# cloneofsimo/paint-with-words-sd

Measured on NVIDIA H100. Metric: unet_steps_per_sec_512sq_cfg, higher is better.
Workload: dtype f16

## Files before the change

include/pww_b200.h:

```cpp
#ifndef PWW_B200_H_
#define PWW_B200_H_

#include <stddef.h>
#include <stdint.h>

#ifdef __cplusplus
extern "C" {
#endif

typedef enum {
  PWW_OK = 0,
  PWW_ERR_BAD_ARG = -1,
  PWW_ERR_UNSUPPORTED = -2,
  PWW_ERR_CUDA = -3,
  PWW_ERR_WORKSPACE = -4
} pww_status_t;

#define PWW_STAT_MAX 0
#define PWW_STAT_STD 1

int pww_version(void);

const char* pww_status_str(int status);

// ... 15 lines not shown
                      int B, int H, int N, int T, int D,
                      int64_t q_batch_stride, int64_t q_row_stride,
                      int64_t k_batch_stride, int64_t k_row_stride,
                      int64_t o_batch_stride, int64_t o_row_stride,
                      const float* wmap, int64_t wmap_batch_stride, const int32_t* wmap_index,
                      const float* stats, const float* g_sigma, float scale, void* stream);

size_t pww_xattn_fused_workspace_bytes(void);
int pww_xattn_fused_f16(const void* q, const void* k, const void* v, void* out,
                        int B, int H, int N, int T, int D,
                        int64_t q_batch_stride, int64_t q_row_stride,
                        int64_t k_batch_stride, int64_t k_row_stride,
                        int64_t o_batch_stride, int64_t o_row_stride,
                        const void* mpack, int64_t mpack_batch_stride, int Bw, const int8_t* cidx,
                        const int32_t* wmap_index, int stat, const float* g_sigma, float scale,
                        float* stats, void* workspace, size_t workspace_bytes, void* stream);

int pww_attn_fwd_f16(const void* q, const void* k, const void* v, void* out,
                     int B, int H, int N, int D,
                     int64_t qkv_batch_stride, int64_t qkv_row_stride,
                     int64_t o_batch_stride, int64_t o_row_stride,
                     float scale, void* stream);

size_t pww_groupnorm_workspace_bytes(int B, int HW, int G);
int pww_groupnorm_nhwc_f16(const void* x, const void* add, int64_t add_batch_stride ,
                           const void* gamma, const void* beta, void* y,
                           int B, int HW, int C, int G, float eps, int silu,
                           void* workspace, size_t workspace_bytes, void* stream);

int pww_geglu_f16(const void* in, void* out, int64_t M, int I, void* stream);

int pww_add_layernorm_f16(const void* x, const void* res, const void* gamma, const void* beta, void* sum_out, void* y,
                          int64_t M, int C, float eps, void* stream);

#ifdef __cplusplus
}
#endif
#endif
```

paint_with_words_sd_b200/__init__.py:

```python
from .attention import PwWAttnProcessor, inj_forward, patch_unet, unpatch_all
from .conditioning import (
    _blur_image_mask, _encode_text_color_inputs, _extract_seed_and_sigma_from_context, _get_binary_mask,
    _image_context_seperator, _img_importance_flatten, _tokens_img_attention_weight, always_round,
)
from .pipeline import (
    PaintWithWord_StableDiffusionInpaintPipeline, PaintWithWord_StableDiffusionPipeline, PwWSampler, paint_with_words,
    paint_with_words_inpaint, preprocess, prepare_mask_and_masked_image, pww_load_tools,
)
from .scheduler import LMSDiscreteScheduler
from .weight_function import UnsupportedWeightFunction, WeightFunction, probe_weight_function

__version__ = "0.1.0"
```

paint_with_words_sd_b200/_native.py:

```python
from __future__ import annotations

import ctypes
import os
from typing import Optional

_HERE = os.path.dirname(os.path.abspath(__file__))
LIB_PATH = os.environ.get("PWW_B200_LIB", os.path.join(_HERE, "libpww_b200.so"))

PWW_STAT_MAX, PWW_STAT_STD = 0, 1

EXPORTS = (
    "pww_version", "pww_status_str", "pww_last_cuda_error", "pww_device_supported",
    "pww_xattn_workspace_bytes", "pww_xattn_stats_f16", "pww_xattn_fwd_f16", "pww_attn_fwd_f16",
    "pww_xattn_fused_workspace_bytes", "pww_xattn_fused_f16",
    "pww_groupnorm_workspace_bytes", "pww_groupnorm_nhwc_f16", "pww_geglu_f16", "pww_add_layernorm_f16",
)


class NativeError(RuntimeError):
    pass


_lib: Optional[ctypes.CDLL] = None
launch_count = 0


def lib() -> ctypes.CDLL:
    global _lib
    if _lib is not None:
        return _lib
    if not os.path.exists(LIB_PATH):
        raise NativeError(
            f"{LIB_PATH} not found: build it with `python -m paint_with_words_sd_b200.csrc.build` "
            "(there is no CPU / PyTorch fallback for the attention path)")
    L = ctypes.CDLL(LIB_PATH)
    c_i, c_i64, c_vp, c_f, c_sz = ctypes.c_int, ctypes.c_int64, ctypes.c_void_p, ctypes.c_float, ctypes.c_size_t
    L.pww_version.restype = c_i
    L.pww_status_str.restype = ctypes.c_char_p
    L.pww_status_str.argtypes = [c_i]
    L.pww_last_cuda_error.restype = ctypes.c_char_p
    L.pww_device_supported.restype = c_i
    L.pww_xattn_workspace_bytes.restype = c_sz
    L.pww_xattn_workspace_bytes.argtypes = [c_i] * 5
    L.pww_xattn_stats_f16.restype = c_i
    L.pww_xattn_stats_f16.argtypes = [c_vp, c_vp, c_i, c_i, c_i, c_i, c_i, c_i64, c_i64, c_i64, c_i64, c_i, c_vp,
                                      c_vp, c_vp, c_sz, c_vp]
    L.pww_xattn_fwd_f16.restype = c_i
    L.pww_xattn_fwd_f16.argtypes = [c_vp, c_vp, c_vp, c_vp, c_i, c_i, c_i, c_i, c_i, c_i64, c_i64, c_i64, c_i64,
                                    c_i64, c_i64, c_vp, c_i64, c_vp, c_vp, c_vp, c_f, c_vp]
    L.pww_xattn_fused_workspace_bytes.restype = c_sz
    L.pww_xattn_fused_workspace_bytes.argtypes = []
    L.pww_xattn_fused_f16.restype = c_i
    L.pww_xattn_fused_f16.argtypes = [c_vp, c_vp, c_vp, c_vp, c_i, c_i, c_i, c_i, c_i, c_i64, c_i64, c_i64, c_i64,
                                      c_i64, c_i64, c_vp, c_i64, c_i, c_vp, c_vp, c_i, c_vp, c_f, c_vp, c_vp, c_sz, c_vp]
    L.pww_attn_fwd_f16.restype = c_i
    L.pww_attn_fwd_f16.argtypes = [c_vp, c_vp, c_vp, c_vp, c_i, c_i, c_i, c_i, c_i64, c_i64, c_i64, c_i64, c_f, c_vp]
    L.pww_groupnorm_workspace_bytes.restype = c_sz
    L.pww_groupnorm_workspace_bytes.argtypes = [c_i, c_i, c_i]
    L.pww_groupnorm_nhwc_f16.restype = c_i
    L.pww_groupnorm_nhwc_f16.argtypes = [c_vp, c_vp, c_i64, c_vp, c_vp, c_vp, c_i, c_i, c_i, c_i, c_f, c_i, c_vp, c_sz, c_vp]
    L.pww_geglu_f16.restype = c_i
    L.pww_geglu_f16.argtypes = [c_vp, c_vp, c_i64, c_i, c_vp]
    L.pww_add_layernorm_f16.restype = c_i
    L.pww_add_layernorm_f16.argtypes = [c_vp, c_vp, c_vp, c_vp, c_vp, c_vp, c_i64, c_i, c_f, c_vp]
    _lib = L
    return L


def check(status: int, what: str) -> None:
    if status != 0:
        L = lib()
        msg = L.pww_status_str(status).decode()
        if status == -3:
            msg += ": " + L.pww_last_cuda_error().decode()
        raise NativeError(f"{what} failed: {msg} (status {status})")
```

paint_with_words_sd_b200/csrc/pww_abi.cu:

```cuda
#include <stdio.h>
#include <string.h>

#include "pww_common.cuh"
#include "xattn_tc.cuh"
#include "xattn_fused.cuh"
#include "xattn_fused2.cuh"
#include "attn_tc.cuh"
#include "unet_ops.cuh"
#include <stdlib.h>

namespace {

thread_local char g_last_cuda_error[640] = "";

int cuda_fail(cudaError_t e);

bool aligned16(const void* p) { return (reinterpret_cast<uintptr_t>(p) & 15u) == 0; }

bool supported_head_dim(int D) { return D == 40 || D == 64 || D == 80 || D == 160; }

int check_common(const void* q, const void* k, int B, int H, int N, int T, int D, int64_t q_bs, int64_t q_rs,
                 int64_t k_bs, int64_t k_rs) {
  if (!q || !k || B <= 0 || H <= 0 || N <= 0 || T <= 0 || D <= 0) return PWW_ERR_BAD_ARG;
  if (!aligned16(q) || !aligned16(k)) return PWW_ERR_BAD_ARG;
  if ((q_bs | q_rs | k_bs | k_rs) & 7) return PWW_ERR_BAD_ARG;
  if (q_rs < (int64_t)H * D || k_rs < (int64_t)H * D) return PWW_ERR_BAD_ARG;
  if (!supported_head_dim(D) || T > pww::tc::kTP) return PWW_ERR_UNSUPPORTED;
  return PWW_OK;
}

size_t align_up(size_t x, size_t a) { return (x + a - 1) / a * a; }

int stats_slots_per_image(int, int) { return 2048; }

int cuda_fail(cudaError_t e) {
  snprintf(g_last_cuda_error, sizeof(g_last_cuda_error), "%s: %s %s", cudaGetErrorName(e), cudaGetErrorString(e),
           pww::tc::tc_error_buf());
  pww::tc::tc_error_buf()[0] = 0;
  return PWW_ERR_CUDA;
}

}

extern "C" {

int pww_version(void) { return 100; }

const char* pww_status_str(int status) {
  switch (status) {
    case PWW_OK: return "ok";
    case PWW_ERR_BAD_ARG: return "bad argument (null/misaligned pointer, non-positive size or stride not a multiple of 8)";
    case PWW_ERR_UNSUPPORTED: return "unsupported shape (head dim must be 40/64/80/160, T <= 80)";
    case PWW_ERR_CUDA: return "CUDA error (see pww_last_cuda_error)";
    case PWW_ERR_WORKSPACE: return "workspace too small (see pww_xattn_workspace_bytes)";
    default: return "unknown status";
  }
}

const char* pww_last_cuda_error(void) { return g_last_cuda_error; }

int pww_device_supported(void) {
  int dev = 0, major = 0;
  cudaError_t e = cudaGetDevice(&dev);
  if (e != cudaSuccess) return cuda_fail(e);
  e = cudaDeviceGetAttribute(&major, cudaDevAttrComputeCapabilityMajor, dev);
  if (e != cudaSuccess) return cuda_fail(e);
  return major == 9 ? 1 : 0;
}

// ... 134 lines not shown
    const void* mp = mpack;
    const int8_t* ci = cidx;
    if (mpack && wmap_index) {
      c.wmap_index = wmap_index + b0;
    } else if (mpack) {
      c.wmap_index = nullptr;
      mp = (const __half*)mpack + (int64_t)b0 * mpack_batch_stride;
      ci = cidx + (int64_t)b0 * pww::fx::kTP;
    }
    c.wmap = mpack ? (const float*)mp : nullptr;
    cudaError_t e = cudaErrorInvalidValue;
    switch (D) {
      case 40: e = pww::fx2::launch_fused2<40>(c, mp, mpack_batch_stride, ci, s); break;
      case 64: e = pww::fx2::launch_fused2<64>(c, mp, mpack_batch_stride, ci, s); break;
      case 80: e = pww::fx2::launch_fused2<80>(c, mp, mpack_batch_stride, ci, s); break;
      case 160: e = pww::fx2::launch_fused2<160>(c, mp, mpack_batch_stride, ci, s); break;
    }
    if (e == cudaErrorInvalidConfiguration) return PWW_ERR_UNSUPPORTED;
    if (e != cudaSuccess) return cuda_fail(e);
  }
  return PWW_OK;
}

size_t pww_groupnorm_workspace_bytes(int B, int HW, int G) {
  if (B <= 0 || HW <= 0 || G <= 0) return 0;
  return align_up((size_t)B * sizeof(unsigned int), 256) + align_up((size_t)B * G * 2 * sizeof(float), 256) +
         (size_t)B * pww::uops::gn_chunks(HW) * G * 2 * sizeof(float);
}

int pww_groupnorm_nhwc_f16(const void* x, const void* add, int64_t add_batch_stride, const void* gamma, const void* beta,
                           void* y, int B, int HW, int C, int G, float eps, int silu, void* workspace,
                           size_t workspace_bytes, void* stream) {
  if (!x || !gamma || !beta || !y || !workspace || B <= 0 || HW <= 0 || C <= 0 || G <= 0) return PWW_ERR_BAD_ARG;
  if (!aligned16(x) || !aligned16(y) || !aligned16(gamma) || !aligned16(beta) || (add && !aligned16(add)))
    return PWW_ERR_BAD_ARG;
  if ((C & 7) || (C % G) || G > 64 || (C >> 3) > 1024) return PWW_ERR_UNSUPPORTED;
  if (add && ((add_batch_stride & 7) || add_batch_stride < C)) return PWW_ERR_BAD_ARG;
  if (workspace_bytes < pww_groupnorm_workspace_bytes(B, HW, G)) return PWW_ERR_WORKSPACE;
  pww::uops::GnParams p;
  p.x = (const __half*)x; p.add = (const __half*)add; p.add_bs = add_batch_stride; p.gamma = (const __half*)gamma; p.beta = (const __half*)beta;
  p.y = (__half*)y;
  char* w = (char*)workspace;
  p.counters = (unsigned int*)w;
  w += align_up((size_t)B * sizeof(unsigned int), 256);
  p.stats = (float*)w;
  w += align_up((size_t)B * G * 2 * sizeof(float), 256);
  p.partial = (float*)w;
  p.B = B; p.HW = HW; p.C = C; p.G = G; p.eps = eps; p.silu = silu;
  p.chunks = pww::uops::gn_chunks(HW);
  p.rows_per_chunk = (HW + p.chunks - 1) / p.chunks;
  cudaStream_t s = (cudaStream_t)stream;
  const int nvec = C >> 3;
  const int rpp = nvec >= 256 ? 1 : 256 / nvec;
  const size_t smem1 = (size_t)rpp * C * 2 * sizeof(float);
  if (smem1 > 48 * 1024) return PWW_ERR_UNSUPPORTED;
  pww::uops::gn_stats_kernel<<<dim3(p.chunks, B), nvec * rpp, smem1, s>>>(p);
  int rows_per_block = (int)(((long long)HW * B + 2 * pww::tc::num_sms() - 1) / (2 * pww::tc::num_sms()));
  if (rows_per_block < rpp) rows_per_block = rpp;
  if (rows_per_block > 32) rows_per_block = 32;
  pww::uops::gn_apply_kernel<<<dim3((HW + rows_per_block - 1) / rows_per_block, B), nvec * rpp, 0, s>>>(p, rows_per_block);
  cudaError_t e = cudaGetLastError();
  return e == cudaSuccess ? PWW_OK : cuda_fail(e);
}

int pww_geglu_f16(const void* in, void* out, int64_t M, int I, void* stream) {
  if (!in || !out || M <= 0 || I <= 0 || !aligned16(in) || !aligned16(out)) return PWW_ERR_BAD_ARG;
  if (I & 7) return PWW_ERR_UNSUPPORTED;
  const long long total = (long long)M * (I >> 3);
  long long blocks = (total + 255) / 256;
  const long long cap = (long long)pww::tc::num_sms() * 16;
  if (blocks > cap) blocks = cap;
  pww::uops::geglu_kernel<<<(int)blocks, 256, 0, (cudaStream_t)stream>>>((const __half*)in, (__half*)out, M, I);
  cudaError_t e = cudaGetLastError();
  return e == cudaSuccess ? PWW_OK : cuda_fail(e);
}

int pww_add_layernorm_f16(const void* x, const void* res, const void* gamma, const void* beta, void* sum_out, void* y,
                          int64_t M, int C, float eps, void* stream) {
  if (!x || !gamma || !beta || !y || M <= 0 || C <= 0) return PWW_ERR_BAD_ARG;
  if (!aligned16(x) || !aligned16(y) || !aligned16(gamma) || !aligned16(beta) || (res && !aligned16(res)) ||
      (sum_out && !aligned16(sum_out)))
    return PWW_ERR_BAD_ARG;
  if ((C & 7) || C > 2048) return PWW_ERR_UNSUPPORTED;
// ... 65 lines not shown
```

paint_with_words_sd_b200/csrc/unet_ops.cuh:

```cuda
#pragma once
#include "pww_common.cuh"

namespace pww {
namespace uops {

struct GnParams {
  const __half* x;
  const __half* add;
  long long add_bs;
  const __half* gamma;
  const __half* beta;
  __half* y;
  float* partial;
  float* stats;
  unsigned int* counters;
  int B, HW, C, G, chunks, rows_per_chunk, silu;
  float eps;
};

__global__ void gn_stats_kernel(GnParams p) {
  extern __shared__ float sm[];
  const int nvec = p.C >> 3;
  const int rpp = blockDim.x / nvec;
  const int v = threadIdx.x % nvec, rl = threadIdx.x / nvec;
  const int b = blockIdx.y, chunk = blockIdx.x;
  const int r0 = chunk * p.rows_per_chunk, r1 = min(p.HW, r0 + p.rows_per_chunk);
  float s[8], q[8], a[8];
#pragma unroll
  for (int i = 0; i < 8; ++i) { s[i] = 0.f; q[i] = 0.f; a[i] = 0.f; }
  if (p.add) {
    const uint4 av = *reinterpret_cast<const uint4*>(p.add + (size_t)b * p.add_bs + v * 8);
    const __half2* ah = reinterpret_cast<const __half2*>(&av);
#pragma unroll
    for (int i = 0; i < 4; ++i) { float2 f = __half22float2(ah[i]); a[2 * i] = f.x; a[2 * i + 1] = f.y; }
  }
  const __half* xb = p.x + (size_t)b * p.HW * p.C;
  for (int r = r0 + rl; r < r1; r += 4 * rpp) {
    uint4 xv[4];
#pragma unroll
    for (int u = 0; u < 4; ++u) {
      const int rr = r + u * rpp;
      xv[u] = rr < r1 ? __ldg(reinterpret_cast<const uint4*>(xb + (size_t)rr * p.C) + v) : make_uint4(0, 0, 0, 0);
    }
#pragma unroll
    for (int u = 0; u < 4; ++u) {
      if (r + u * rpp < r1) {
        const __half2* xh = reinterpret_cast<const __half2*>(&xv[u]);
#pragma unroll
        for (int i = 0; i < 4; ++i) {
          float2 f = __half22float2(xh[i]);
          const float x0 = f.x + a[2 * i], x1 = f.y + a[2 * i + 1];
          s[2 * i] += x0; q[2 * i] = fmaf(x0, x0, q[2 * i]);
          s[2 * i + 1] += x1; q[2 * i + 1] = fmaf(x1, x1, q[2 * i + 1]);
        }
      }
    }
  }
  float* ss = sm;
  float* sq = sm + rpp * p.C;
#pragma unroll
  for (int i = 0; i < 8; ++i) { ss[rl * p.C + v * 8 + i] = s[i]; sq[rl * p.C + v * 8 + i] = q[i]; }
  __syncthreads();
  const int cg = p.C / p.G;
  for (int g = threadIdx.x; g < p.G; g += blockDim.x) {
    float ts = 0.f, tq = 0.f;
    for (int r = 0; r < rpp; ++r)
      for (int c = g * cg; c < (g + 1) * cg; ++c) { ts += ss[r * p.C + c]; tq += sq[r * p.C + c]; }
    float* out = p.partial + (((size_t)b * p.chunks + chunk) * p.G + g) * 2;
    out[0] = ts; out[1] = tq;
  }
  __shared__ int is_last;
  __threadfence();
  __syncthreads();
  if (threadIdx.x == 0) is_last = (atomicAdd(&p.counters[b], 1u) == (unsigned)p.chunks - 1u) ? 1 : 0;
  __syncthreads();
  if (!is_last) return;
  __threadfence();
  const int warp = threadIdx.x >> 5, lane = threadIdx.x & 31, nwarps = blockDim.x >> 5;
  for (int g = warp; warp < nwarps && g < p.G; g += nwarps) {
    const float* pp = p.partial + ((size_t)b * p.chunks * p.G + g) * 2;
    float ts = 0.f, tq = 0.f;
    for (int c = lane; c < p.chunks; c += 32) { ts += __ldcg(pp + (size_t)c * p.G * 2); tq += __ldcg(pp + (size_t)c * p.G * 2 + 1); }
#pragma unroll
    for (int o = 16; o > 0; o >>= 1) {
      ts += __shfl_xor_sync(0xffffffffu, ts, o);
      tq += __shfl_xor_sync(0xffffffffu, tq, o);
    }
    if (lane == 0) {
      const float n = (float)p.HW * (float)cg;
      const float mean = ts / n;
      float var = tq / n - mean * mean;
      var = var < 0.f ? 0.f : var;
      p.stats[((size_t)b * p.G + g) * 2] = mean;
      p.stats[((size_t)b * p.G + g) * 2 + 1] = rsqrtf(var + p.eps);
    }
  }
  if (threadIdx.x == 0) p.counters[b] = 0u;
}

__global__ void gn_apply_kernel(GnParams p, int rows_per_block) {
  const int nvec = p.C >> 3;
  const int rpp = blockDim.x / nvec;
  const int v = threadIdx.x % nvec, rl = threadIdx.x / nvec;
  const int b = blockIdx.y;
  const int cg = p.C / p.G;
  float sc[8], sh[8];
  {
    const uint4 gv = __ldg(reinterpret_cast<const uint4*>(p.gamma) + v);
    const uint4 bv = __ldg(reinterpret_cast<const uint4*>(p.beta) + v);
    uint4 av = make_uint4(0, 0, 0, 0);
    if (p.add) av = __ldg(reinterpret_cast<const uint4*>(p.add + (size_t)b * p.add_bs) + v);
    const __half* gh = reinterpret_cast<const __half*>(&gv);
    const __half* bh = reinterpret_cast<const __half*>(&bv);
    const __half* ah = reinterpret_cast<const __half*>(&av);
#pragma unroll
    for (int i = 0; i < 8; ++i) {
      const int g = (v * 8 + i) / cg;
      const float mean = __ldg(p.stats + ((size_t)b * p.G + g) * 2), rstd = __ldg(p.stats + ((size_t)b * p.G + g) * 2 + 1);
      sc[i] = rstd * __half2float(gh[i]);
      sh[i] = __half2float(bh[i]) + (__half2float(ah[i]) - mean) * sc[i];
    }
  }
  const int r0 = blockIdx.x * rows_per_block, r1 = min(p.HW, r0 + rows_per_block);
  const __half* xb = p.x + (size_t)b * p.HW * p.C;
  __half* yb = p.y + (size_t)b * p.HW * p.C;
  for (int r = r0 + rl; r < r1; r += rpp) {
    const uint4 xv = __ldg(reinterpret_cast<const uint4*>(xb + (size_t)r * p.C) + v);
    const __half2* xh = reinterpret_cast<const __half2*>(&xv);
    __align__(16) __half2 o[4];
#pragma unroll
    for (int k = 0; k < 4; ++k) {
      const float2 f = __half22float2(xh[k]);
      float y0 = fmaf(f.x, sc[2 * k], sh[2 * k]);
      float y1 = fmaf(f.y, sc[2 * k + 1], sh[2 * k + 1]);
      if (p.silu) {
        y0 = __fdividef(y0, 1.f + __expf(-y0));
        y1 = __fdividef(y1, 1.f + __expf(-y1));
      }
      o[k] = __floats2half2_rn(y0, y1);
    }
    reinterpret_cast<uint4*>(yb + (size_t)r * p.C)[v] = *reinterpret_cast<const uint4*>(o);
  }
}

__global__ void geglu_kernel(const __half* __restrict__ in, __half* __restrict__ out, long long M, int I) {
  const int nvec = I >> 3;
  const long long total = M * nvec;
  for (long long i = (long long)blockIdx.x * blockDim.x + threadIdx.x; i < total; i += (long long)gridDim.x * blockDim.x) {
    const long long m = i / nvec;
    const int v = (int)(i % nvec);
    const uint4 av = __ldg(reinterpret_cast<const uint4*>(in + m * 2 * I) + v);
    const uint4 gv = __ldg(reinterpret_cast<const uint4*>(in + m * 2 * I + I) + v);
    const __half2* ah = reinterpret_cast<const __half2*>(&av);
    const __half2* gh = reinterpret_cast<const __half2*>(&gv);
    __align__(16) __half2 o[4];
#pragma unroll
    for (int k = 0; k < 4; ++k) {
      const float2 a = __half22float2(ah[k]), g = __half22float2(gh[k]);
      const float g0 = 0.5f * g.x * (1.f + erff(g.x * 0.70710678118654752f));
      const float g1 = 0.5f * g.y * (1.f + erff(g.y * 0.70710678118654752f));
      o[k] = __floats2half2_rn(a.x * g0, a.y * g1);
    }
    reinterpret_cast<uint4*>(out + m * I)[v] = *reinterpret_cast<const uint4*>(o);
  }
}

template <int VPL>
// ... 43 lines not shown
  }
#pragma unroll
  for (int o = 16; o > 0; o >>= 1) sq += __shfl_xor_sync(0xffffffffu, sq, o);
  const float rstd = rsqrtf(sq / (float)C + eps);
#pragma unroll
  for (int i = 0; i < VPL; ++i) {
    const int vi = lane + i * 32;
    if (vi < nvec) {
      const uint4 gv = __ldg(reinterpret_cast<const uint4*>(gamma) + vi);
      const uint4 bv = __ldg(reinterpret_cast<const uint4*>(beta) + vi);
      const __half2* gh = reinterpret_cast<const __half2*>(&gv);
      const __half2* bh = reinterpret_cast<const __half2*>(&bv);
      __align__(16) __half2 o[4];
#pragma unroll
      for (int k = 0; k < 4; ++k) {
        const float2 g = __half22float2(gh[k]), b = __half22float2(bh[k]);
        o[k] = __floats2half2_rn((v[i][2 * k] - mean) * rstd * g.x + b.x, (v[i][2 * k + 1] - mean) * rstd * g.y + b.y);
      }
      reinterpret_cast<uint4*>(y + row * C)[vi] = *reinterpret_cast<const uint4*>(o);
    }
  }
}

inline int gn_chunks(int HW) {
  int rows = HW >= 4096 ? 64 : (HW >= 1024 ? 32 : 16);
  int c = (HW + rows - 1) / rows;
  return c < 1 ? 1 : (c > 512 ? 512 : c);
}

}
}
```

paint_with_words_sd_b200/fused_ops.py:

```python
from __future__ import annotations

from typing import Dict, Optional

import torch

from . import _native

_WS: Dict[torch.device, torch.Tensor] = {}


def _workspace(device, nbytes: int) -> torch.Tensor:
    w = _WS.get(device)
    if w is None or w.numel() < nbytes:
        if w is not None:
            _WS_KEEP.append(w)
        w = torch.zeros(max(nbytes, 4 << 20), dtype=torch.uint8, device=device)
        _WS[device] = w
    return w


_WS_KEEP: list = []


ENABLED = True


def is_fast(x: torch.Tensor) -> bool:
    return ENABLED and x.is_cuda and x.dtype == torch.float16


def group_norm_nhwc(x: torch.Tensor, gn: torch.nn.GroupNorm, add: Optional[torch.Tensor] = None,
                    silu: bool = True) -> torch.Tensor:
    if not x.is_contiguous(memory_format=torch.channels_last):
        x = x.contiguous(memory_format=torch.channels_last)
    B, C, H, W = x.shape
    L = _native.lib()
    y = torch.empty_like(x, memory_format=torch.channels_last)
    nbytes = L.pww_groupnorm_workspace_bytes(B, H * W, gn.num_groups)
    ws = _workspace(x.device, nbytes)
    add_bs = 0
    if add is not None:
        if add.dtype != torch.float16 or add.stride(-1) != 1 or (add.stride(0) % 8) or (add.data_ptr() % 16):
            add = add.to(torch.float16).contiguous()
        add_bs = add.stride(0)
    with torch.cuda.device(x.device):
        rc = L.pww_groupnorm_nhwc_f16(x.data_ptr(), None if add is None else add.data_ptr(), add_bs, gn.weight.data_ptr(),
                                      gn.bias.data_ptr(), y.data_ptr(), B, H * W, C, gn.num_groups, float(gn.eps),
                                      1 if silu else 0, ws.data_ptr(), ws.numel(),
                                      torch.cuda.current_stream(x.device).cuda_stream)
    _native.check(rc, "pww_groupnorm_nhwc_f16")
    _native.launch_count += 2
    return y


def geglu(h: torch.Tensor) -> torch.Tensor:
    if not h.is_contiguous():
        h = h.contiguous()
    I = h.shape[-1] // 2
    M = h.numel() // h.shape[-1]
    out = torch.empty(h.shape[:-1] + (I,), dtype=h.dtype, device=h.device)
    with torch.cuda.device(h.device):
        rc = _native.lib().pww_geglu_f16(h.data_ptr(), out.data_ptr(), M, I, torch.cuda.current_stream(h.device).cuda_stream)
    _native.check(rc, "pww_geglu_f16")
    _native.launch_count += 1
    return out


def add_layer_norm(x: torch.Tensor, res: Optional[torch.Tensor], ln: torch.nn.LayerNorm, want_sum: bool = True):
    if not x.is_contiguous():
        x = x.contiguous()
    if res is not None and not res.is_contiguous():
        res = res.contiguous()
    C = x.shape[-1]
    M = x.numel() // C
    y = torch.empty_like(x)
# ... 10 lines not shown
```

paint_with_words_sd_b200/unet.py:

```python
from __future__ import annotations

import math
from dataclasses import dataclass, field
from typing import List, Optional, Sequence, Tuple, Union

import torch
import torch.nn as nn
import torch.nn.functional as F

from . import fused_ops


@dataclass
class UNetConfig:
    in_channels: int = 4
    out_channels: int = 4
    block_out_channels: Tuple[int, ...] = (320, 640, 1280, 1280)
    layers_per_block: int = 2
    cross_attention_dim: int = 768
    attention_heads: Union[int, Tuple[int, ...]] = 8
    use_linear_projection: bool = False
    norm_num_groups: int = 32
    sample_size: int = 64

# ... 115 lines not shown
        wo = self.proj_out.weight
        t = F.linear(t, wo.reshape(wo.shape[0], wo.shape[1]), self.proj_out.bias) + res
        return t.reshape(b, h, w, c).permute(0, 3, 1, 2)

    def forward(self, x, encoder_hidden_states=None):
        if fused_ops.is_fast(x):
            return self._forward_fast(x, encoder_hidden_states)
        b, c, h, w = x.shape
        res = x
        x = self.norm(x)
        if self.linear_proj:
            x = self.proj_in(x.permute(0, 2, 3, 1).reshape(b, h * w, c))
        else:
            x = self.proj_in(x).permute(0, 2, 3, 1).reshape(b, h * w, -1)
        for blk in self.transformer_blocks:
            x = blk(x, context=encoder_hidden_states)
        if self.linear_proj:
            x = self.proj_out(x).reshape(b, h, w, c).permute(0, 3, 1, 2)
        else:
            x = self.proj_out(x.reshape(b, h, w, -1).permute(0, 3, 1, 2))
        return x + res


class ResnetBlock2D(nn.Module):
    def __init__(self, in_ch, out_ch, temb_ch, groups):
        super().__init__()
        self.norm1 = nn.GroupNorm(groups, in_ch, eps=1e-5)
        self.conv1 = nn.Conv2d(in_ch, out_ch, 3, padding=1)
        self.time_emb_proj = nn.Linear(temb_ch, out_ch)
        self.norm2 = nn.GroupNorm(groups, out_ch, eps=1e-5)
        self.conv2 = nn.Conv2d(out_ch, out_ch, 3, padding=1)
        self.conv_shortcut = nn.Conv2d(in_ch, out_ch, 1) if in_ch != out_ch else None

    def forward(self, x, temb):
        if fused_ops.is_fast(x):
            h = self.conv1(fused_ops.group_norm_nhwc(x, self.norm1, silu=True))
            t = getattr(self, "_pww_t", None)
            if t is None:
                t = self.time_emb_proj(F.silu(temb))
            h = self.conv2(fused_ops.group_norm_nhwc(h, self.norm2, add=t, silu=True))
            return (x if self.conv_shortcut is None else self.conv_shortcut(x)) + h
        h = self.conv1(F.silu(self.norm1(x)))
        h = h + self.time_emb_proj(F.silu(temb))[:, :, None, None]
        h = self.conv2(F.silu(self.norm2(h)))
        return (x if self.conv_shortcut is None else self.conv_shortcut(x)) + h


class Downsample2D(nn.Module):
    def __init__(self, ch):
        super().__init__()
        self.conv = nn.Conv2d(ch, ch, 3, stride=2, padding=1)

    def forward(self, x):
        return self.conv(x)


class Upsample2D(nn.Module):
    def __init__(self, ch):
        super().__init__()
        self.conv = nn.Conv2d(ch, ch, 3, padding=1)

    def forward(self, x):
        return self.conv(F.interpolate(x, scale_factor=2.0, mode="nearest"))

# ... 121 lines not shown
        if fast:
            x = x.contiguous(memory_format=torch.channels_last)
            self._project_time_embeddings(temb)
        x = self.conv_in(x)
        skips = [x]
        for blk in self.down_blocks:
            x, outs = blk(x, temb, encoder_hidden_states)
            skips.extend(outs)
        x = self.mid_block(x, temb, encoder_hidden_states)
        for blk in self.up_blocks:
            x = blk(x, skips, temb, encoder_hidden_states)
        if fast:
            x = self.conv_out(fused_ops.group_norm_nhwc(x, self.conv_norm_out, silu=True))
        else:
            x = self.conv_out(F.silu(self.conv_norm_out(x)))
        return _Sample(x)


def _resnets(unet: nn.Module):
    return [m for m in unet.modules() if isinstance(m, ResnetBlock2D)]


def _project_time_embeddings(self, temb):
    cache = self.__dict__.get("_pww_temb_w")
    res = _resnets(self)
    if cache is None or cache[0].device != temb.device or cache[0].dtype != temb.dtype:
        w = torch.cat([r.time_emb_proj.weight for r in res], 0).detach().contiguous()
        b = torch.cat([r.time_emb_proj.bias for r in res], 0).detach().contiguous()
        cache = (w, b)
        self.__dict__["_pww_temb_w"] = cache
    t_all = F.linear(F.silu(temb), cache[0], cache[1])
    off = 0
    for r in res:
        n = r.time_emb_proj.weight.shape[0]
        object.__setattr__(r, "_pww_t", t_all[:, off:off + n])
        off += n


UNet2DConditionModel._project_time_embeddings = _project_time_embeddings


def attention_modules(unet: nn.Module):
    return [m for m in unet.modules() if m.__class__.__name__ == "CrossAttention"]


def build_unet(cfg: UNetConfig, seed: int = 0, dtype=torch.float32, device="cpu") -> UNet2DConditionModel:
    with torch.random.fork_rng(devices=[]):
        torch.manual_seed(seed)
        unet = UNet2DConditionModel(cfg)
    unet.eval().requires_grad_(False)
    unet = unet.to(device=device, dtype=dtype)
    if torch.device(device).type == "cuda":
        unet = unet.to(memory_format=torch.channels_last)
    return unet
# ... 1 lines not shown
```

Before: 129.9.

## Fuse GroupNorm into single cluster kernel and fold conv biases into residual add

GroupNorm now runs as one thread-block-cluster kernel. Each cluster reduces a channel slab's statistics through distributed shared memory and can keep the slab cached in shared memory for the apply pass, replacing the separate stats and apply launches and the global workspace. The ResNet block drops the conv biases: conv1's bias is folded into the time-embedding bias, and conv2's and the shortcut's biases are added in a new fused residual-plus-bias kernel. This cuts launches and extra passes over memory, at the cost of more complex cluster code, a mean-shifted variance computation, and a per-call cache key built over every parameter in Python.

```diff
diff --git a/include/pww_b200.h b/include/pww_b200.h
--- a/include/pww_b200.h
+++ b/include/pww_b200.h
@@ -61,11 +61,12 @@
                      int64_t o_batch_stride, int64_t o_row_stride,
                      float scale, void* stream);
 
-size_t pww_groupnorm_workspace_bytes(int B, int HW, int G);
 int pww_groupnorm_nhwc_f16(const void* x, const void* add, int64_t add_batch_stride ,
                            const void* gamma, const void* beta, void* y,
-                           int B, int HW, int C, int G, float eps, int silu,
-                           void* workspace, size_t workspace_bytes, void* stream);
+                           int B, int HW, int C, int G, float eps, int silu, void* stream);
+
+int pww_residual_bias_add_f16(const void* a, const void* b, const void* bias0, const void* bias1, void* out,
+                              int64_t M, int C, void* stream);
 
 int pww_geglu_f16(const void* in, void* out, int64_t M, int I, void* stream);
 
diff --git a/paint_with_words_sd_b200/__init__.py b/paint_with_words_sd_b200/__init__.py
--- a/paint_with_words_sd_b200/__init__.py
+++ b/paint_with_words_sd_b200/__init__.py
@@ -10,4 +10,4 @@
 from .scheduler import LMSDiscreteScheduler
 from .weight_function import UnsupportedWeightFunction, WeightFunction, probe_weight_function
 
-__version__ = "0.1.0"
+__version__ = "0.2.0"
diff --git a/paint_with_words_sd_b200/_native.py b/paint_with_words_sd_b200/_native.py
--- a/paint_with_words_sd_b200/_native.py
+++ b/paint_with_words_sd_b200/_native.py
@@ -13,7 +13,7 @@
     "pww_version", "pww_status_str", "pww_last_cuda_error", "pww_device_supported",
     "pww_xattn_workspace_bytes", "pww_xattn_stats_f16", "pww_xattn_fwd_f16", "pww_attn_fwd_f16",
     "pww_xattn_fused_workspace_bytes", "pww_xattn_fused_f16",
-    "pww_groupnorm_workspace_bytes", "pww_groupnorm_nhwc_f16", "pww_geglu_f16", "pww_add_layernorm_f16",
+    "pww_groupnorm_nhwc_f16", "pww_residual_bias_add_f16", "pww_geglu_f16", "pww_add_layernorm_f16",
 )
 
 
@@ -55,10 +55,10 @@
                                       c_i64, c_i64, c_vp, c_i64, c_i, c_vp, c_vp, c_i, c_vp, c_f, c_vp, c_vp, c_sz, c_vp]
     L.pww_attn_fwd_f16.restype = c_i
     L.pww_attn_fwd_f16.argtypes = [c_vp, c_vp, c_vp, c_vp, c_i, c_i, c_i, c_i, c_i64, c_i64, c_i64, c_i64, c_f, c_vp]
-    L.pww_groupnorm_workspace_bytes.restype = c_sz
-    L.pww_groupnorm_workspace_bytes.argtypes = [c_i, c_i, c_i]
     L.pww_groupnorm_nhwc_f16.restype = c_i
-    L.pww_groupnorm_nhwc_f16.argtypes = [c_vp, c_vp, c_i64, c_vp, c_vp, c_vp, c_i, c_i, c_i, c_i, c_f, c_i, c_vp, c_sz, c_vp]
+    L.pww_groupnorm_nhwc_f16.argtypes = [c_vp, c_vp, c_i64, c_vp, c_vp, c_vp, c_i, c_i, c_i, c_i, c_f, c_i, c_vp]
+    L.pww_residual_bias_add_f16.restype = c_i
+    L.pww_residual_bias_add_f16.argtypes = [c_vp, c_vp, c_vp, c_vp, c_vp, c_i64, c_i, c_vp]
     L.pww_geglu_f16.restype = c_i
     L.pww_geglu_f16.argtypes = [c_vp, c_vp, c_i64, c_i, c_vp]
     L.pww_add_layernorm_f16.restype = c_i
diff --git a/paint_with_words_sd_b200/csrc/pww_abi.cu b/paint_with_words_sd_b200/csrc/pww_abi.cu
--- a/paint_with_words_sd_b200/csrc/pww_abi.cu
+++ b/paint_with_words_sd_b200/csrc/pww_abi.cu
@@ -44,7 +44,7 @@
 
 extern "C" {
 
-int pww_version(void) { return 100; }
+int pww_version(void) { return 200; }
 
 const char* pww_status_str(int status) {
   switch (status) {
@@ -225,43 +225,57 @@
   return PWW_OK;
 }
 
-size_t pww_groupnorm_workspace_bytes(int B, int HW, int G) {
-  if (B <= 0 || HW <= 0 || G <= 0) return 0;
-  return align_up((size_t)B * sizeof(unsigned int), 256) + align_up((size_t)B * G * 2 * sizeof(float), 256) +
-         (size_t)B * pww::uops::gn_chunks(HW) * G * 2 * sizeof(float);
-}
-
 int pww_groupnorm_nhwc_f16(const void* x, const void* add, int64_t add_batch_stride, const void* gamma, const void* beta,
-                           void* y, int B, int HW, int C, int G, float eps, int silu, void* workspace,
-                           size_t workspace_bytes, void* stream) {
-  if (!x || !gamma || !beta || !y || !workspace || B <= 0 || HW <= 0 || C <= 0 || G <= 0) return PWW_ERR_BAD_ARG;
+                           void* y, int B, int HW, int C, int G, float eps, int silu, void* stream) {
+  if (!x || !gamma || !beta || !y || B <= 0 || HW <= 0 || C <= 0 || G <= 0) return PWW_ERR_BAD_ARG;
   if (!aligned16(x) || !aligned16(y) || !aligned16(gamma) || !aligned16(beta) || (add && !aligned16(add)))
     return PWW_ERR_BAD_ARG;
-  if ((C & 7) || (C % G) || G > 64 || (C >> 3) > 1024) return PWW_ERR_UNSUPPORTED;
+  if ((C & 7) || (C % G) || G > 64 || (C >> 3) > 1024 || B > 65535) return PWW_ERR_UNSUPPORTED;
   if (add && ((add_batch_stride & 7) || add_batch_stride < C)) return PWW_ERR_BAD_ARG;
-  if (workspace_bytes < pww_groupnorm_workspace_bytes(B, HW, G)) return PWW_ERR_WORKSPACE;
+  if ((C / G) / pww::uops::gn_gcd(C / G, 8) > pww::uops::kGnMaxThreads) return PWW_ERR_UNSUPPORTED;
+  static int smem_optin[pww::tc::kMaxDevices] = {0};
+  const int dev = pww::tc::cur_device();
+  if (!smem_optin[dev]) {
+    int v = 0;
+    cudaError_t e = cudaDeviceGetAttribute(&v, cudaDevAttrMaxSharedMemoryPerBlockOptin, dev);
+    v -= 2 * 2 * pww::uops::kGnMaxGroupsPerSlab * (int)sizeof(float);
+    if (e == cudaSuccess) e = cudaFuncSetAttribute(pww::uops::gn_fused_kernel, cudaFuncAttributeMaxDynamicSharedMemorySize, v);
+    if (e != cudaSuccess) return cuda_fail(e);
+    smem_optin[dev] = v;
+  }
+  const pww::uops::GnPlan g = pww::uops::gn_plan(HW, C, G, smem_optin[dev]);
+  if (g.smem_bytes > (size_t)smem_optin[dev]) return PWW_ERR_UNSUPPORTED;
   pww::uops::GnParams p;
   p.x = (const __half*)x; p.add = (const __half*)add; p.add_bs = add_batch_stride; p.gamma = (const __half*)gamma; p.beta = (const __half*)beta;
   p.y = (__half*)y;
-  char* w = (char*)workspace;
-  p.counters = (unsigned int*)w;
-  w += align_up((size_t)B * sizeof(unsigned int), 256);
-  p.stats = (float*)w;
-  w += align_up((size_t)B * G * 2 * sizeof(float), 256);
-  p.partial = (float*)w;
-  p.B = B; p.HW = HW; p.C = C; p.G = G; p.eps = eps; p.silu = silu;
-  p.chunks = pww::uops::gn_chunks(HW);
-  p.rows_per_chunk = (HW + p.chunks - 1) / p.chunks;
-  cudaStream_t s = (cudaStream_t)stream;
-  const int nvec = C >> 3;
-  const int rpp = nvec >= 256 ? 1 : 256 / nvec;
-  const size_t smem1 = (size_t)rpp * C * 2 * sizeof(float);
-  if (smem1 > 48 * 1024) return PWW_ERR_UNSUPPORTED;
-  pww::uops::gn_stats_kernel<<<dim3(p.chunks, B), nvec * rpp, smem1, s>>>(p);
-  int rows_per_block = (int)(((long long)HW * B + 2 * pww::tc::num_sms() - 1) / (2 * pww::tc::num_sms()));
-  if (rows_per_block < rpp) rows_per_block = rpp;
-  if (rows_per_block > 32) rows_per_block = 32;
-  pww::uops::gn_apply_kernel<<<dim3((HW + rows_per_block - 1) / rows_per_block, B), nvec * rpp, 0, s>>>(p, rows_per_block);
+  p.HW = HW; p.C = C; p.cg = C / G; p.S = g.S; p.rpp = g.rpp; p.rows_per_cta = g.rows_per_cta;
+  p.cached = g.cached ? 1 : 0; p.silu = silu; p.eps = eps;
+  cudaLaunchConfig_t cfg;
+  memset(&cfg, 0, sizeof(cfg));
+  cfg.gridDim = dim3(g.cluster * (C / g.S), B);
+  cfg.blockDim = dim3(g.threads);
+  cfg.dynamicSmemBytes = g.smem_bytes;
+  cfg.stream = (cudaStream_t)stream;
+  cudaLaunchAttribute attr[1];
+  attr[0].id = cudaLaunchAttributeClusterDimension;
+  attr[0].val.clusterDim.x = g.cluster; attr[0].val.clusterDim.y = 1; attr[0].val.clusterDim.z = 1;
+  cfg.attrs = attr; cfg.numAttrs = 1;
+  cudaError_t e = cudaLaunchKernelEx(&cfg, pww::uops::gn_fused_kernel, p);
+  return e == cudaSuccess ? PWW_OK : cuda_fail(e);
+}
+
+int pww_residual_bias_add_f16(const void* a, const void* b, const void* bias0, const void* bias1, void* out, int64_t M,
+                              int C, void* stream) {
+  if (!a || !b || !bias0 || !out || M <= 0 || C <= 0) return PWW_ERR_BAD_ARG;
+  if (!aligned16(a) || !aligned16(b) || !aligned16(bias0) || (bias1 && !aligned16(bias1)) || !aligned16(out))
+    return PWW_ERR_BAD_ARG;
+  if (C & 7) return PWW_ERR_UNSUPPORTED;
+  const long long total = (long long)M * (C >> 3);
+  long long blocks = (total + 255) / 256;
+  const long long cap = (long long)pww::tc::num_sms() * 16;
+  if (blocks > cap) blocks = cap;
+  pww::uops::residual_bias_add_kernel<<<(int)blocks, 256, 0, (cudaStream_t)stream>>>(
+      (const __half*)a, (const __half*)b, (const __half*)bias0, (const __half*)bias1, (__half*)out, M, C);
   cudaError_t e = cudaGetLastError();
   return e == cudaSuccess ? PWW_OK : cuda_fail(e);
 }
diff --git a/paint_with_words_sd_b200/csrc/unet_ops.cuh b/paint_with_words_sd_b200/csrc/unet_ops.cuh
--- a/paint_with_words_sd_b200/csrc/unet_ops.cuh
+++ b/paint_with_words_sd_b200/csrc/unet_ops.cuh
@@ -1,8 +1,16 @@
 #pragma once
+#include <cooperative_groups.h>
+
 #include "pww_common.cuh"
 
 namespace pww {
 namespace uops {
+
+constexpr int kGnMaxCluster = 8;
+constexpr int kGnMaxGroupsPerSlab = 8;
+constexpr int kGnCtaBytes = 32 * 1024;
+constexpr int kGnRowsPerThread = 8;
+constexpr int kGnMaxThreads = 512;
 
 struct GnParams {
   const __half* x;
@@ -11,121 +19,161 @@
   const __half* gamma;
   const __half* beta;
   __half* y;
-  float* partial;
-  float* stats;
-  unsigned int* counters;
-  int B, HW, C, G, chunks, rows_per_chunk, silu;
+  int HW, C, cg;
+  int S, rpp;
+  int rows_per_cta;
+  int cached;
+  int silu;
   float eps;
 };
 
-__global__ void gn_stats_kernel(GnParams p) {
-  extern __shared__ float sm[];
-  const int nvec = p.C >> 3;
-  const int rpp = blockDim.x / nvec;
-  const int v = threadIdx.x % nvec, rl = threadIdx.x / nvec;
-  const int b = blockIdx.y, chunk = blockIdx.x;
-  const int r0 = chunk * p.rows_per_chunk, r1 = min(p.HW, r0 + p.rows_per_chunk);
-  float s[8], q[8], a[8];
-#pragma unroll
-  for (int i = 0; i < 8; ++i) { s[i] = 0.f; q[i] = 0.f; a[i] = 0.f; }
-  if (p.add) {
-    const uint4 av = *reinterpret_cast<const uint4*>(p.add + (size_t)b * p.add_bs + v * 8);
-    const __half2* ah = reinterpret_cast<const __half2*>(&av);
-#pragma unroll
-    for (int i = 0; i < 4; ++i) { float2 f = __half22float2(ah[i]); a[2 * i] = f.x; a[2 * i + 1] = f.y; }
-  }
-  const __half* xb = p.x + (size_t)b * p.HW * p.C;
-  for (int r = r0 + rl; r < r1; r += 4 * rpp) {
-    uint4 xv[4];
-#pragma unroll
-    for (int u = 0; u < 4; ++u) {
-      const int rr = r + u * rpp;
-      xv[u] = rr < r1 ? __ldg(reinterpret_cast<const uint4*>(xb + (size_t)rr * p.C) + v) : make_uint4(0, 0, 0, 0);
-    }
-#pragma unroll
-    for (int u = 0; u < 4; ++u) {
-      if (r + u * rpp < r1) {
-        const __half2* xh = reinterpret_cast<const __half2*>(&xv[u]);
-#pragma unroll
-        for (int i = 0; i < 4; ++i) {
-          float2 f = __half22float2(xh[i]);
-          const float x0 = f.x + a[2 * i], x1 = f.y + a[2 * i + 1];
-          s[2 * i] += x0; q[2 * i] = fmaf(x0, x0, q[2 * i]);
-          s[2 * i + 1] += x1; q[2 * i + 1] = fmaf(x1, x1, q[2 * i + 1]);
-        }
-      }
-    }
-  }
-  float* ss = sm;
-  float* sq = sm + rpp * p.C;
-#pragma unroll
-  for (int i = 0; i < 8; ++i) { ss[rl * p.C + v * 8 + i] = s[i]; sq[rl * p.C + v * 8 + i] = q[i]; }
+__device__ __forceinline__ void gn_group_sums(const GnParams& p, const float (&acc0)[8], const float (&acc1)[8],
+                                              float* red, float (*out)[kGnMaxGroupsPerSlab]) {
+  const int nvs = p.S >> 3;
+  const int v = threadIdx.x % nvs, rl = threadIdx.x / nvs;
+  const int J = max(1, (int)blockDim.x / p.S);
+  const int RS = p.rpp * p.S;
+  float* red2 = red + 2 * RS;
+#pragma unroll
+  for (int i = 0; i < 8; ++i) {
+    red[rl * p.S + v * 8 + i] = acc0[i];
+    red[RS + rl * p.S + v * 8 + i] = acc1[i];
+  }
   __syncthreads();
-  const int cg = p.C / p.G;
-  for (int g = threadIdx.x; g < p.G; g += blockDim.x) {
-    float ts = 0.f, tq = 0.f;
-    for (int r = 0; r < rpp; ++r)
-      for (int c = g * cg; c < (g + 1) * cg; ++c) { ts += ss[r * p.C + c]; tq += sq[r * p.C + c]; }
-    float* out = p.partial + (((size_t)b * p.chunks + chunk) * p.G + g) * 2;
-    out[0] = ts; out[1] = tq;
-  }
-  __shared__ int is_last;
-  __threadfence();
+  for (int w = threadIdx.x; w < 2 * J * p.S; w += blockDim.x) {
+    const int q = w / (J * p.S), jc = w % (J * p.S);
+    const int c = jc % p.S, j = jc / p.S;
+    const float* src = red + q * RS;
+    float t = 0.f;
+    for (int r = j; r < p.rpp; r += J) t += src[r * p.S + c];
+    red2[w] = t;
+  }
   __syncthreads();
-  if (threadIdx.x == 0) is_last = (atomicAdd(&p.counters[b], 1u) == (unsigned)p.chunks - 1u) ? 1 : 0;
+  for (int w = threadIdx.x; w < 2 * p.S; w += blockDim.x) {
+    const int q = w / p.S, c = w % p.S;
+    float t = 0.f;
+    for (int j = 0; j < J; ++j) t += red2[(q * J + j) * p.S + c];
+    red[w] = t;
+  }
   __syncthreads();
-  if (!is_last) return;
-  __threadfence();
   const int warp = threadIdx.x >> 5, lane = threadIdx.x & 31, nwarps = blockDim.x >> 5;
-  for (int g = warp; warp < nwarps && g < p.G; g += nwarps) {
-    const float* pp = p.partial + ((size_t)b * p.chunks * p.G + g) * 2;
-    float ts = 0.f, tq = 0.f;
-    for (int c = lane; c < p.chunks; c += 32) { ts += __ldcg(pp + (size_t)c * p.G * 2); tq += __ldcg(pp + (size_t)c * p.G * 2 + 1); }
-#pragma unroll
-    for (int o = 16; o > 0; o >>= 1) {
-      ts += __shfl_xor_sync(0xffffffffu, ts, o);
-      tq += __shfl_xor_sync(0xffffffffu, tq, o);
-    }
-    if (lane == 0) {
-      const float n = (float)p.HW * (float)cg;
-      const float mean = ts / n;
-      float var = tq / n - mean * mean;
-      var = var < 0.f ? 0.f : var;
-      p.stats[((size_t)b * p.G + g) * 2] = mean;
-      p.stats[((size_t)b * p.G + g) * 2 + 1] = rsqrtf(var + p.eps);
-    }
-  }
-  if (threadIdx.x == 0) p.counters[b] = 0u;
-}
-
-__global__ void gn_apply_kernel(GnParams p, int rows_per_block) {
-  const int nvec = p.C >> 3;
-  const int rpp = blockDim.x / nvec;
-  const int v = threadIdx.x % nvec, rl = threadIdx.x / nvec;
-  const int b = blockIdx.y;
-  const int cg = p.C / p.G;
+  const int gs = p.S / p.cg;
+  for (int w = warp; warp < nwarps && w < 2 * gs; w += nwarps) {
+    const int q = w / gs, g = w % gs;
+    float t = 0.f;
+    for (int c = lane; c < p.cg; c += 32) t += red[q * p.S + g * p.cg + c];
+#pragma unroll
+    for (int o = 16; o > 0; o >>= 1) t += __shfl_xor_sync(0xffffffffu, t, o);
+    if (lane == 0) out[q][g] = t;
+  }
+}
+
+__device__ __forceinline__ void gn_cluster_sums(const float* part, int gs, int ncl, float (&tot)[kGnMaxGroupsPerSlab]) {
+  namespace cgr = cooperative_groups;
+  cgr::cluster_group cluster = cgr::this_cluster();
+  const int lane = threadIdx.x & 31;
+  const float* src = lane >= ncl ? nullptr : (ncl == 1 ? part : cluster.map_shared_rank(part, lane));
+#pragma unroll
+  for (int g = 0; g < kGnMaxGroupsPerSlab; ++g) tot[g] = (src && g < gs) ? src[g] : 0.f;
+#pragma unroll
+  for (int g = 0; g < kGnMaxGroupsPerSlab; ++g)
+#pragma unroll
+    for (int o = kGnMaxCluster / 2; o > 0; o >>= 1) tot[g] += __shfl_xor_sync(0xffffffffu, tot[g], o);
+}
+
+__global__ void __launch_bounds__(kGnMaxThreads) gn_fused_kernel(GnParams p) {
+  namespace cgr = cooperative_groups;
+  cgr::cluster_group cluster = cgr::this_cluster();
+  extern __shared__ __align__(16) unsigned char gn_smem[];
+  __shared__ float part[2][kGnMaxGroupsPerSlab];
+  __shared__ float stat[2][kGnMaxGroupsPerSlab];
+  const int nvs = p.S >> 3;
+  const int v = threadIdx.x % nvs, rl = threadIdx.x / nvs;
+  const int ncl = (int)cluster.num_blocks(), rank = (int)cluster.block_rank();
+  const int b = blockIdx.y, c0 = (blockIdx.x / ncl) * p.S;
+  const int gs = p.S / p.cg;
+  const int r0 = rank * p.rows_per_cta, r1 = min(p.HW, r0 + p.rows_per_cta);
+  const int J = max(1, (int)blockDim.x / p.S);
+  float* red = reinterpret_cast<float*>(gn_smem);
+  uint4* cache = p.cached ? reinterpret_cast<uint4*>(gn_smem + (size_t)2 * (p.rpp + J) * p.S * sizeof(float)) : nullptr;
+  const __half* xi = p.x + (size_t)b * p.HW * p.C + c0;
+  const __half* xb = xi + v * 8;
+  const __half* ai = p.add ? p.add + (size_t)b * p.add_bs + c0 : nullptr;
+  const float n = (float)p.HW * (float)p.cg;
+
+  float ak[8];
+  {
+    uint4 av = make_uint4(0, 0, 0, 0);
+    if (ai) av = __ldg(reinterpret_cast<const uint4*>(ai) + v);
+    const __half* ah = reinterpret_cast<const __half*>(&av);
+#pragma unroll
+    for (int i = 0; i < 8; ++i) {
+      const int f = (v * 8 + i) / p.cg * p.cg;
+      const float k = __half2float(__ldg(xi + f)) + (ai ? __half2float(__ldg(ai + f)) : 0.f);
+      ak[i] = __half2float(ah[i]) - k;
+    }
+  }
+  auto for_rows = [&](const uint4* src, auto&& f) {
+    for (int r = r0 + rl; r < r1; r += 4 * p.rpp) {
+      uint4 xv[4];
+#pragma unroll
+      for (int u = 0; u < 4; ++u) {
+        const int rr = r + u * p.rpp;
+        xv[u] = rr >= r1 ? make_uint4(0, 0, 0, 0)
+                         : (src ? src[(size_t)(rr - r0) * nvs + v] : __ldg(reinterpret_cast<const uint4*>(xb + (size_t)rr * p.C)));
+      }
+#pragma unroll
+      for (int u = 0; u < 4; ++u)
+        if (r + u * p.rpp < r1) f(xv[u], r + u * p.rpp);
+    }
+  };
+
+  float s1[8], s2[8];
+#pragma unroll
+  for (int i = 0; i < 8; ++i) { s1[i] = 0.f; s2[i] = 0.f; }
+  for_rows(nullptr, [&](const uint4& xv, int rr) {
+    if (cache) cache[(size_t)(rr - r0) * nvs + v] = xv;
+    const __half2* xh = reinterpret_cast<const __half2*>(&xv);
+#pragma unroll
+    for (int k = 0; k < 4; ++k) {
+      const float2 f = __half22float2(xh[k]);
+      const float d0 = f.x + ak[2 * k], d1 = f.y + ak[2 * k + 1];
+      s1[2 * k] += d0; s2[2 * k] = fmaf(d0, d0, s2[2 * k]);
+      s1[2 * k + 1] += d1; s2[2 * k + 1] = fmaf(d1, d1, s2[2 * k + 1]);
+    }
+  });
+  gn_group_sums(p, s1, s2, red, part);
+  if (ncl > 1) cluster.sync(); else __syncthreads();
+  if (threadIdx.x < 32) {
+    float t1[kGnMaxGroupsPerSlab], t2[kGnMaxGroupsPerSlab];
+    gn_cluster_sums(&part[0][0], gs, ncl, t1);
+    gn_cluster_sums(&part[1][0], gs, ncl, t2);
+#pragma unroll
+    for (int g = 0; g < kGnMaxGroupsPerSlab; ++g)
+      if (threadIdx.x == g) {
+        const float m = t1[g] / n;
+        stat[0][g] = m;
+        stat[1][g] = rsqrtf(fmaxf(t2[g] / n - m * m, 0.f) + p.eps);
+      }
+  }
+  if (ncl > 1) cluster.barrier_arrive();
+  __syncthreads();
+
   float sc[8], sh[8];
   {
-    const uint4 gv = __ldg(reinterpret_cast<const uint4*>(p.gamma) + v);
-    const uint4 bv = __ldg(reinterpret_cast<const uint4*>(p.beta) + v);
-    uint4 av = make_uint4(0, 0, 0, 0);
-    if (p.add) av = __ldg(reinterpret_cast<const uint4*>(p.add + (size_t)b * p.add_bs) + v);
+    const uint4 gv = __ldg(reinterpret_cast<const uint4*>(p.gamma + c0) + v);
+    const uint4 bv = __ldg(reinterpret_cast<const uint4*>(p.beta + c0) + v);
     const __half* gh = reinterpret_cast<const __half*>(&gv);
     const __half* bh = reinterpret_cast<const __half*>(&bv);
-    const __half* ah = reinterpret_cast<const __half*>(&av);
 #pragma unroll
     for (int i = 0; i < 8; ++i) {
-      const int g = (v * 8 + i) / cg;
-      const float mean = __ldg(p.stats + ((size_t)b * p.G + g) * 2), rstd = __ldg(p.stats + ((size_t)b * p.G + g) * 2 + 1);
-      sc[i] = rstd * __half2float(gh[i]);
-      sh[i] = __half2float(bh[i]) + (__half2float(ah[i]) - mean) * sc[i];
-    }
-  }
-  const int r0 = blockIdx.x * rows_per_block, r1 = min(p.HW, r0 + rows_per_block);
-  const __half* xb = p.x + (size_t)b * p.HW * p.C;
-  __half* yb = p.y + (size_t)b * p.HW * p.C;
-  for (int r = r0 + rl; r < r1; r += rpp) {
-    const uint4 xv = __ldg(reinterpret_cast<const uint4*>(xb + (size_t)r * p.C) + v);
+      const int g = (v * 8 + i) / p.cg;
+      sc[i] = stat[1][g] * __half2float(gh[i]);
+      sh[i] = __half2float(bh[i]) + (ak[i] - stat[0][g]) * sc[i];
+    }
+  }
+  __half* yb = p.y + (size_t)b * p.HW * p.C + c0 + v * 8;
+  for_rows(cache, [&](const uint4& xv, int rr) {
     const __half2* xh = reinterpret_cast<const __half2*>(&xv);
     __align__(16) __half2 o[4];
 #pragma unroll
@@ -139,10 +187,34 @@
       }
       o[k] = __floats2half2_rn(y0, y1);
     }
-    reinterpret_cast<uint4*>(yb + (size_t)r * p.C)[v] = *reinterpret_cast<const uint4*>(o);
-  }
-}
-
+    *reinterpret_cast<uint4*>(yb + (size_t)rr * p.C) = *reinterpret_cast<const uint4*>(o);
+  });
+  if (ncl > 1) cluster.barrier_wait();
+}
+
+__global__ void residual_bias_add_kernel(const __half* __restrict__ a, const __half* __restrict__ b,
+                                         const __half* __restrict__ bias0, const __half* __restrict__ bias1,
+                                         __half* __restrict__ out, long long M, int C) {
+  const int nvec = C >> 3;
+  const long long total = M * nvec;
+  for (long long i = (long long)blockIdx.x * blockDim.x + threadIdx.x; i < total; i += (long long)gridDim.x * blockDim.x) {
+    const int v = (int)(i % nvec);
+    const uint4 av = __ldg(reinterpret_cast<const uint4*>(a) + i);
+    const uint4 bv = __ldg(reinterpret_cast<const uint4*>(b) + i);
+    const uint4 cv = __ldg(reinterpret_cast<const uint4*>(bias0) + v);
+    const uint4 dv = bias1 ? __ldg(reinterpret_cast<const uint4*>(bias1) + v) : make_uint4(0, 0, 0, 0);
+    const __half2 *ah = reinterpret_cast<const __half2*>(&av), *bh = reinterpret_cast<const __half2*>(&bv);
+    const __half2 *ch = reinterpret_cast<const __half2*>(&cv), *dh = reinterpret_cast<const __half2*>(&dv);
+    __align__(16) __half2 o[4];
+#pragma unroll
+    for (int k = 0; k < 4; ++k) {
+      const float2 x = __half22float2(ah[k]), y = __half22float2(bh[k]);
+      const float2 c = __half22float2(ch[k]), d = __half22float2(dh[k]);
+      o[k] = __floats2half2_rn((x.x + y.x) + (c.x + d.x), (x.y + y.y) + (c.y + d.y));
+    }
+    reinterpret_cast<uint4*>(out)[i] = *reinterpret_cast<const uint4*>(o);
+  }
+}
 __global__ void geglu_kernel(const __half* __restrict__ in, __half* __restrict__ out, long long M, int I) {
   const int nvec = I >> 3;
   const long long total = M * nvec;
@@ -232,11 +304,35 @@
   }
 }
 
-inline int gn_chunks(int HW) {
-  int rows = HW >= 4096 ? 64 : (HW >= 1024 ? 32 : 16);
-  int c = (HW + rows - 1) / rows;
-  return c < 1 ? 1 : (c > 512 ? 512 : c);
-}
-
-}
-}
+inline int gn_gcd(int a, int b) { return b ? gn_gcd(b, a % b) : a; }
+
+struct GnPlan {
+  int S, rpp, threads, cluster, rows_per_cta;
+  bool cached;
+  size_t red_bytes, cache_bytes, smem_bytes;
+};
+
+inline GnPlan gn_plan(int HW, int C, int G, int smem_optin) {
+  GnPlan g;
+  const int cgc = C / G;
+  g.S = cgc / gn_gcd(cgc, 8) * 8;
+  const int nvs = g.S >> 3;
+  const long long slab_bytes = (long long)HW * g.S * (long long)sizeof(__half);
+  g.cluster = (int)((slab_bytes + kGnCtaBytes - 1) / kGnCtaBytes);
+  if (g.cluster > kGnMaxCluster) g.cluster = kGnMaxCluster;
+  g.rows_per_cta = (HW + g.cluster - 1) / g.cluster;
+  g.rpp = (g.rows_per_cta + kGnRowsPerThread - 1) / kGnRowsPerThread;
+  const int max_rpp = kGnMaxThreads / nvs;
+  if (g.rpp > max_rpp) g.rpp = max_rpp;
+  if (g.rpp * nvs < 32) g.rpp = (32 + nvs - 1) / nvs;
+  g.threads = nvs * g.rpp;
+  const int J = g.threads / g.S > 1 ? g.threads / g.S : 1;
+  g.red_bytes = (size_t)2 * (g.rpp + J) * g.S * sizeof(float);
+  g.cache_bytes = (size_t)g.rows_per_cta * g.S * sizeof(__half);
+  g.cached = g.red_bytes + g.cache_bytes <= (size_t)smem_optin / 2;
+  g.smem_bytes = g.red_bytes + (g.cached ? g.cache_bytes : 0);
+  return g;
+}
+
+}
+}
diff --git a/paint_with_words_sd_b200/fused_ops.py b/paint_with_words_sd_b200/fused_ops.py
--- a/paint_with_words_sd_b200/fused_ops.py
+++ b/paint_with_words_sd_b200/fused_ops.py
@@ -1,26 +1,10 @@
 from __future__ import annotations
 
-from typing import Dict, Optional
+from typing import Optional
 
 import torch
 
 from . import _native
-
-_WS: Dict[torch.device, torch.Tensor] = {}
-
-
-def _workspace(device, nbytes: int) -> torch.Tensor:
-    w = _WS.get(device)
-    if w is None or w.numel() < nbytes:
-        if w is not None:
-            _WS_KEEP.append(w)
-        w = torch.zeros(max(nbytes, 4 << 20), dtype=torch.uint8, device=device)
-        _WS[device] = w
-    return w
-
-
-_WS_KEEP: list = []
-
 
 ENABLED = True
 
@@ -36,8 +20,6 @@
     B, C, H, W = x.shape
     L = _native.lib()
     y = torch.empty_like(x, memory_format=torch.channels_last)
-    nbytes = L.pww_groupnorm_workspace_bytes(B, H * W, gn.num_groups)
-    ws = _workspace(x.device, nbytes)
     add_bs = 0
     if add is not None:
         if add.dtype != torch.float16 or add.stride(-1) != 1 or (add.stride(0) % 8) or (add.data_ptr() % 16):
@@ -46,11 +28,39 @@
     with torch.cuda.device(x.device):
         rc = L.pww_groupnorm_nhwc_f16(x.data_ptr(), None if add is None else add.data_ptr(), add_bs, gn.weight.data_ptr(),
                                       gn.bias.data_ptr(), y.data_ptr(), B, H * W, C, gn.num_groups, float(gn.eps),
-                                      1 if silu else 0, ws.data_ptr(), ws.numel(),
-                                      torch.cuda.current_stream(x.device).cuda_stream)
+                                      1 if silu else 0, torch.cuda.current_stream(x.device).cuda_stream)
     _native.check(rc, "pww_groupnorm_nhwc_f16")
-    _native.launch_count += 2
+    _native.launch_count += 1
     return y
+
+
+def _bias_f16(t: torch.Tensor, C: int, device) -> torch.Tensor:
+    if t.numel() != C:
+        raise ValueError(f"bias has {t.numel()} elements, expected {C}")
+    if t.dtype != torch.float16 or t.device != device or not t.is_contiguous() or t.data_ptr() % 16:
+        t = t.to(device=device, dtype=torch.float16).contiguous()
+    return t
+
+
+def residual_bias_add(a: torch.Tensor, b: torch.Tensor, bias0: torch.Tensor,
+                      bias1: Optional[torch.Tensor] = None) -> torch.Tensor:
+    if a.shape != b.shape:
+        raise ValueError(f"residual_bias_add: shapes differ {tuple(a.shape)} vs {tuple(b.shape)}")
+    if not a.is_contiguous(memory_format=torch.channels_last):
+        a = a.contiguous(memory_format=torch.channels_last)
+    if not b.is_contiguous(memory_format=torch.channels_last):
+        b = b.contiguous(memory_format=torch.channels_last)
+    C = b.shape[1]
+    bias0 = _bias_f16(bias0, C, b.device)
+    bias1 = None if bias1 is None else _bias_f16(bias1, C, b.device)
+    out = torch.empty_like(b, memory_format=torch.channels_last)
+    with torch.cuda.device(b.device):
+        rc = _native.lib().pww_residual_bias_add_f16(a.data_ptr(), b.data_ptr(), bias0.data_ptr(),
+                                                     None if bias1 is None else bias1.data_ptr(), out.data_ptr(),
+                                                     b.numel() // C, C, torch.cuda.current_stream(b.device).cuda_stream)
+    _native.check(rc, "pww_residual_bias_add_f16")
+    _native.launch_count += 1
+    return out
 
 
 def geglu(h: torch.Tensor) -> torch.Tensor:
diff --git a/paint_with_words_sd_b200/unet.py b/paint_with_words_sd_b200/unet.py
--- a/paint_with_words_sd_b200/unet.py
+++ b/paint_with_words_sd_b200/unet.py
@@ -161,6 +161,10 @@
         return x + res
 
 
+def _conv_no_bias(conv: nn.Conv2d, x: torch.Tensor) -> torch.Tensor:
+    return F.conv2d(x, conv.weight, None, conv.stride, conv.padding, conv.dilation, conv.groups)
+
+
 class ResnetBlock2D(nn.Module):
     def __init__(self, in_ch, out_ch, temb_ch, groups):
         super().__init__()
@@ -173,12 +177,15 @@
 
     def forward(self, x, temb):
         if fused_ops.is_fast(x):
-            h = self.conv1(fused_ops.group_norm_nhwc(x, self.norm1, silu=True))
+            h = _conv_no_bias(self.conv1, fused_ops.group_norm_nhwc(x, self.norm1, silu=True))
             t = getattr(self, "_pww_t", None)
             if t is None:
-                t = self.time_emb_proj(F.silu(temb))
-            h = self.conv2(fused_ops.group_norm_nhwc(h, self.norm2, add=t, silu=True))
-            return (x if self.conv_shortcut is None else self.conv_shortcut(x)) + h
+                t = F.linear(F.silu(temb), self.time_emb_proj.weight, self.time_emb_proj.bias + self.conv1.bias)
+            h = _conv_no_bias(self.conv2, fused_ops.group_norm_nhwc(h, self.norm2, add=t, silu=True))
+            if self.conv_shortcut is None:
+                return fused_ops.residual_bias_add(x, h, self.conv2.bias)
+            return fused_ops.residual_bias_add(_conv_no_bias(self.conv_shortcut, x), h, self.conv2.bias,
+                                               self.conv_shortcut.bias)
         h = self.conv1(F.silu(self.norm1(x)))
         h = h + self.time_emb_proj(F.silu(temb))[:, :, None, None]
         h = self.conv2(F.silu(self.norm2(h)))
@@ -346,14 +353,16 @@
 
 
 def _project_time_embeddings(self, temb):
+    res = _resnets(self)
+    params = [p for r in res for p in (r.time_emb_proj.weight, r.time_emb_proj.bias, r.conv1.bias)]
+    key = tuple((p.data_ptr(), p._version, p.dtype, p.device) for p in params)
     cache = self.__dict__.get("_pww_temb_w")
-    res = _resnets(self)
-    if cache is None or cache[0].device != temb.device or cache[0].dtype != temb.dtype:
+    if cache is None or cache[0] != key:
         w = torch.cat([r.time_emb_proj.weight for r in res], 0).detach().contiguous()
-        b = torch.cat([r.time_emb_proj.bias for r in res], 0).detach().contiguous()
-        cache = (w, b)
+        b = torch.cat([r.time_emb_proj.bias + r.conv1.bias for r in res], 0).detach().contiguous()
+        cache = (key, w, b)
         self.__dict__["_pww_temb_w"] = cache
-    t_all = F.linear(F.silu(temb), cache[0], cache[1])
+    t_all = F.linear(F.silu(temb), cache[1], cache[2])
     off = 0
     for r in res:
         n = r.time_emb_proj.weight.shape[0]
```

New measurement: 135.5, median of 6. +4.3%, better.
